# Limeth/euclider

Hardware: NVIDIA B200
Metric: Mrays/s (higher is better)
Workload: dtype f64

## Files before the change

### euclider_b200/csrc/cuda/api_device.cu

```cuda
#include <algorithm>
#include <cmath>
#include <cstdio>
#include <cstdlib>
#include <cstring>
#include <condition_variable>
#include <functional>
#include <mutex>
#include <string>
#include <thread>
#include <vector>

#include "error.h"
#include "euclider_b200.h"
#include "intersect.cuh"
#include "pipeline.cuh"
#include "scene_dev.cuh"

namespace {

using namespace eucl;

#define EUCL_CUDA(expr)                                                                                   \
    do {                                                                                                  \
        cudaError_t _e = (expr);                                                                          \
// ... 53 lines not shown
            }
        });
    }
    void run(std::function<void()> f) {
        std::lock_guard<std::mutex> lk(m);
        job = std::move(f);
        has_job = true;
        done = false;
        cv.notify_all();
    }
    void wait() {
        std::unique_lock<std::mutex> lk(m);
        cv.wait(lk, [this] { return done; });
    }
    void stop() {
        if (!th.joinable()) return;
        {
            std::lock_guard<std::mutex> lk(m);
            quit = true;
            cv.notify_all();
        }
        th.join();
    }
};

}

struct EuclScene {
    int device = 0;
    int dim = 3;
    int sm_count = 148;
    int blob_bytes = 0;
    size_t smem_bytes = 0;
    size_t smem_scene = 0;
    unsigned long long shade_light_mask = 1ull, shade_heavy_mask = 0ull;
    uint8_t* d_blob = nullptr;
    std::vector<cudaArray_t> arrays;
    std::vector<cudaTextureObject_t> tex_objects;
    cudaStream_t stream = nullptr;
    cudaStream_t own_stream = nullptr;
    cudaEvent_t ev[2] = {nullptr, nullptr};
    cudaStream_t side_stream = nullptr;
    cudaEvent_t ev_fork = nullptr, ev_join = nullptr;
    std::vector<cudaEvent_t> prof_events;
    DeviceBuffer nodes;
    DeviceBuffer small;
    DeviceBuffer frame;
    DeviceBuffer hit_ids;
    DeviceBuffer order;
    DeviceBuffer path_io;
    DeviceBuffer rorder;
    int n_cull = 0;
    int light_capable = 0;
    int ray_bins_mode = -1;
    bool ray_bins_now = true;
    float tune_ms[2] = {0.f, 0.f};
    int tune_count[2] = {0, 0};
    uint64_t tune_pixels = 0;
    int warm_frames = 0;
    int n_entities = 0;
    int real_bytes = 8;
    int arena_capacity = 0;
    double arena_factor = 0.0;
    cudaGraphExec_t graph_exec = nullptr;
    uint64_t graph_key = 0, seen_key = 0;
    uint32_t graph_launches = 0;
    int list_capacity = 0;
    double list_factor = 1.0;
    int32_t* h_small = nullptr;
    std::vector<EuclScene*> twins;
    std::vector<Worker*> workers;
    bool is_twin = false;
    cudaEvent_t ev_split[3] = {nullptr, nullptr, nullptr};
    cudaEvent_t ev_done = nullptr;
};

namespace {

constexpr int kSmallInts = 4 * (EUCL_MAX_LEVELS + 1) + 16 + (EUCL_MAX_LEVELS + 1) * (kMaxBins + kRayBins);
struct SmallLayout {
    static constexpr int count = 0;
    static constexpr int level_off = EUCL_MAX_LEVELS + 1;
    static constexpr int overflow = 2 * (EUCL_MAX_LEVELS + 1);
    static constexpr int cam_entity = overflow + 1;
    static constexpr int undefined64 = overflow + 2;
    static constexpr int mega64 = undefined64 + 2;
    static constexpr int bins = mega64 + 2 * (EUCL_MAX_LEVELS + 1);
    static constexpr int rbins = bins + (EUCL_MAX_LEVELS + 1) * kMaxBins;
    static constexpr int total = rbins + (EUCL_MAX_LEVELS + 1) * kRayBins;
};
static_assert(SmallLayout::undefined64 % 2 == 0, "u64 counters must be 8-byte aligned");
static_assert(SmallLayout::total <= kSmallInts, "small buffer layout");

size_t align16(size_t v) { return (v + 15) & ~size_t(15); }

int validate_scene(const EuclFlatScene& f, std::string* why) {
    auto bad = [&](const std::string& msg) {
        *why = msg;
        return (int)EUCL_ERR_INVALID_ARGUMENT;
    };
    const int counts[] = {f.n_prims, f.n_nodes, f.n_entities, f.n_materials, f.n_transforms, f.n_expr_ops,
                          f.n_surfaces, f.n_color_ops, f.n_mapped_textures, f.n_textures};
    for (int c : counts)
        if (c < 0) return bad("negative table size");
    if ((f.n_prims && !f.prims) || (f.n_nodes && !f.nodes) || (f.n_entities && !f.entities) || (f.n_materials && !f.materials) ||
        (f.n_transforms && !f.transforms) || (f.n_expr_ops && !f.expr_ops) || (f.n_surfaces && !f.surfaces) ||
// ... 561 lines not shown
        for (int k = 0; k < EUCL_MAX_DIM; ++k) planes[(size_t)i * kPlaneStride + k] = flat->prims[i].v0[k];
        planes[(size_t)i * kPlaneStride + 4] = flat->prims[i].s0;
        planes[(size_t)i * kPlaneStride + 5] = flat->prims[i].s1;
    }
    h.off_planes = w.put(planes.data(), planes.size());
    MacroBuilder mb{*flat, {}};
    std::vector<EuclEntity> dev_entities((size_t)flat->n_entities);
    std::vector<char> negated((size_t)std::max(flat->n_entities, 1), 0);
    for (int e = 0; e < flat->n_entities; ++e) {
        EuclEntity de = flat->entities[e];
        de.node_first = (int)mb.out.size();
        const int root = flat->entities[e].node_root;
        const EuclNode& rn = flat->nodes[root];
        if (rn.op == EUCL_CSG_COMPLEMENT && flat->nodes[mb.child_a(root)].op == EUCL_CSG_LEAF &&
            flat->prims[flat->nodes[mb.child_a(root)].prim].kind == EUCL_PRIM_VOID && env_int("EUCL_NEGATED_ROOMS", 1)) {
            negated[(size_t)e] = 1;
            mb.emit(mb.child_b(root));
        } else {
            mb.emit(root);
        }
        de.node_root = (int)mb.out.size() - 1;
        int peak = 0, depth = 0;
        if (!mb.fits(de.node_first, de.node_root, &peak, &depth))
            return bail(EUCL_ERR_SCENE_LIMIT, "entity " + std::to_string(e) + ": CSG program too large for the device evaluator (" +
                                                  std::to_string(peak) + " arena slots of " + std::to_string(CSG_ARENA) + ", nesting " +
                                                  std::to_string(depth) + ")");
        dev_entities[(size_t)e] = de;
    }
    std::vector<Bound> bounds(mb.out.size());
    for (int e = 0; e < flat->n_entities; ++e)
        mb.compute_bounds(dev_entities[(size_t)e].node_first, dev_entities[(size_t)e].node_root, s->real_bytes == 4 ? 1e-3 : 1e-6, &bounds);
    if (!env_int("EUCL_BOUND_CULL", 1))
        for (auto& b : bounds) b.r2 = -1.0;
    h.n_nodes = (int)mb.out.size();
    h.off_nodes = w.put(mb.out.data(), mb.out.size());
    h.off_bounds = w.put(bounds.data(), bounds.size());
    for (int e = 0; e < flat->n_entities && h.n_cull < 4; ++e) {
        const EuclEntity& de = dev_entities[(size_t)e];
        if (de.surface >= 0 && !negated[(size_t)e] && mb.out[(size_t)de.node_root].kind != M_PRIM && bounds[(size_t)de.node_root].r2 >= 0.0)
            h.cull_root[h.n_cull++] = de.node_root;
    }
    s->n_cull = h.n_cull;
    std::vector<int32_t> ent_flags((size_t)std::max(flat->n_entities, 1), 0);
    bool light_capable = true;
    for (int e = 0; e < flat->n_entities; ++e) {
        const EuclEntity& de = dev_entities[(size_t)e];
        if (negated[(size_t)e]) ent_flags[(size_t)e] = ENT_NEGATED;
        if (de.surface < 0) continue;
        const MNode& root = mb.out[(size_t)de.node_root];
        int fl = ENT_SURFACED | ent_flags[(size_t)e];
        if (root.kind == M_PRIM) fl |= ENT_PRIM;
        else if (root.kind == M_CHAIN && de.node_first == de.node_root && (root.b & 0x4000) && (root.b & 0x3fff) <= kPlaneChainMax) fl |= ENT_ROOT_PLANES;
        for (int k = 0; k < h.n_cull; ++k)
            if (h.cull_root[k] == de.node_root) fl |= ENT_CULL_ROOT;
        if (!(fl & (ENT_PRIM | ENT_ROOT_PLANES | ENT_CULL_ROOT))) light_capable = false;
        ent_flags[(size_t)e] = fl;
    }
    if (!env_int("EUCL_INTERSECT_SPLIT", 1)) light_capable = false;
    h.light_capable = light_capable ? 1 : 0;
    s->light_capable = h.light_capable;
    h.off_ent_flags = w.put(ent_flags.data(), ent_flags.size());
    h.off_entities = w.put(dev_entities.data(), dev_entities.size());
    h.off_materials = w.put(flat->materials, (size_t)flat->n_materials);
    h.off_transforms = w.put(flat->transforms, (size_t)flat->n_transforms);
    h.off_expr_ops = w.put(flat->expr_ops, (size_t)flat->n_expr_ops);
    std::vector<LinRow> lin_rows((size_t)std::max(flat->n_transforms, 1) * 2 * EUCL_MAX_DIM);
    for (int t = 0; t < flat->n_transforms; ++t)
        for (int k = 0; k < flat->dim; ++k) {
            const EuclTransform& tr = flat->transforms[t];
            lin_rows[(size_t)t * 2 * EUCL_MAX_DIM + k] = lower_lin_row(flat->expr_ops + tr.fwd_first[k], tr.fwd_len[k], flat->dim);
            lin_rows[(size_t)t * 2 * EUCL_MAX_DIM + EUCL_MAX_DIM + k] = lower_lin_row(flat->expr_ops + tr.inv_first[k], tr.inv_len[k], flat->dim);
        }
    h.off_lin_rows = w.put(lin_rows.data(), lin_rows.size());
    h.off_surfaces = w.put(flat->surfaces, (size_t)flat->n_surfaces);
    h.off_color_ops = w.put(flat->color_ops, (size_t)flat->n_color_ops);
    h.off_mapped = w.put(flat->mapped_textures, (size_t)flat->n_mapped_textures);
    h.off_textures = w.put(flat->textures, (size_t)flat->n_textures);
    h.off_tex_objects = w.put(s->tex_objects.data(), s->tex_objects.size());
    h.off_perlin = w.put(flat->perlin_perm, 256);
    int max_nodes = 1;
    for (int e = 0; e < flat->n_entities; ++e)
        max_nodes = std::max(max_nodes, flat->entities[e].node_root - flat->entities[e].node_first + 1);
    h.max_entity_nodes = max_nodes;
    h.blob_bytes = (int)w.bytes.size();
    std::memcpy(w.bytes.data(), &h, sizeof h);
    s->blob_bytes = h.blob_bytes;
    s->smem_scene = scene_smem_bytes(h.blob_bytes);
    s->smem_bytes = s->smem_scene + sizeof(double) * kPlaneChainMax * kBlock;
    s->shade_light_mask = 1ull;
    s->shade_heavy_mask = 0ull;
    if (kBinsPerEntity * flat->n_entities + 1 <= kMaxBins)
        for (int e = 0; e < flat->n_entities; ++e) {
            const int sf = flat->entities[e].surface;
            if (sf < 0) continue;
            const bool simple = flat->surfaces[sf].ratio_op == EUCL_RATIO_UNIFORM && flat->surfaces[sf].thr_op == EUCL_THR_IDENTITY;
            const unsigned long long bits = ((1ull << kBinsPerEntity) - 1ull) << (1 + kBinsPerEntity * e);
            (simple ? s->shade_light_mask : s->shade_heavy_mask) |= bits;
        }
    if (env_int("EUCL_SHADE_SPLIT", 1) == 0) {
        s->shade_heavy_mask |= s->shade_light_mask;
        s->shade_light_mask = 0ull;
    }
    int smem_optin = 0;
    cudaDeviceGetAttribute(&smem_optin, cudaDevAttrMaxSharedMemoryPerBlockOptin, device);
    if (s->smem_bytes > (size_t)smem_optin)
        return bail(EUCL_ERR_SCENE_LIMIT, "scene tables (" + std::to_string(s->smem_bytes) +
                                              " B) exceed the shared memory of one CTA (" + std::to_string(smem_optin) + " B)");
    EUCL_CUDA_S(cudaMalloc((void**)&s->d_blob, w.bytes.size()));
    EUCL_CUDA_S(cudaMemcpy(s->d_blob, w.bytes.data(), w.bytes.size(), cudaMemcpyHostToDevice));
    EUCL_CUDA_S(EUCL_PREC(configure_kernels)(s->smem_bytes, s->smem_scene));
    EUCL_CUDA_S(cudaMallocHost((void**)&s->h_small, sizeof(int32_t) * kSmallInts));
#undef EUCL_CUDA_S
    *out = s;
// ... 88 lines not shown
    return ws;
}

void choose_grouping(EuclScene* s) {
    const int forced = env_int("EUCL_BIN_RAYS", -1);
    if (forced >= 0) s->ray_bins_mode = forced ? 1 : 0;
    if (s->ray_bins_mode >= 0) s->ray_bins_now = s->ray_bins_mode == 1;
    else s->ray_bins_now = s->tune_count[1] <= s->tune_count[0];
}

void tune_grouping(EuclScene* s, const EuclStats& st, int pipeline) {
    if (s->ray_bins_mode >= 0 || st.retries != 0 || st.pixels == 0 || pipeline != EUCL_PIPELINE_WAVEFRONT) return;
    if (s->n_cull == 0) {
        s->ray_bins_mode = 0;
    } else if (s->warm_frames >= 1) {
        if (s->tune_pixels != st.pixels) {
            s->tune_pixels = st.pixels;
            s->tune_ms[0] = s->tune_ms[1] = 0.f;
            s->tune_count[0] = s->tune_count[1] = 0;
        }
        const int m = s->ray_bins_now ? 1 : 0;
        s->tune_ms[m] = s->tune_count[m] == 0 ? st.ms_total : std::min(s->tune_ms[m], st.ms_total);
        s->tune_count[m] += 1;
        if (s->tune_count[0] >= 2 && s->tune_count[1] >= 2) s->ray_bins_mode = s->tune_ms[1] < s->tune_ms[0] ? 1 : 0;
    }
}

int render_impl(EuclScene* s, const EuclCamera* cam, const EuclRenderOpts* o, uint8_t* d_rgb, int32_t* d_hit,
                EuclStats* stats, int sub_stride = 1, int sub_offset = 0) {
    const int dim = s->dim;
    FrameParams fp;
    frame_params(*cam, *o, s->real_bytes, &fp);
    const int width = (int)o->width;
    const uint32_t my_rows = eucl_band_rows_for_rank(o);
    EuclStats st{};
    st.levels = cam->max_depth + 1;
    if (!s->is_twin) choose_grouping(s);
    EUCL_CUDA(cudaEventRecord(s->ev[0], s->stream));
    if (my_rows > 0) {
        const long long chunk_pixels_target = std::max(1, env_int("EUCL_CHUNK_PIXELS", 1 << 25));
        int rows_per_chunk = (int)std::max<long long>(1, chunk_pixels_target / width);
        rows_per_chunk = std::min<int>(rows_per_chunk, (int)my_rows);
        if ((long long)width > (1ll << 30)) return fail(EUCL_ERR_INVALID_ARGUMENT, "frame rows too wide");
        EUCL_CUDA(s->small.ensure(sizeof(int32_t) * kSmallInts));
        if (s->arena_factor <= 0.0) s->arena_factor = std::max(1.0, (double)env_int("EUCL_ARENA_FACTOR_X10", 45) / 10.0);
        Launch l{s->stream, s->d_blob, s->smem_bytes, s->smem_scene,
                 s->sm_count * std::max(1, env_int("EUCL_BLOCKS_PER_SM", kResidentThreads / kBlock)),
                 s->sm_count * std::max(1, env_int("EUCL_LIGHT_BLOCKS_PER_SM", kLightResidentBlocks)),
                 s->sm_count * std::max(1, env_int("EUCL_SHADE_BLOCKS_PER_SM", kShadeResidentBlocks)),
                 s->sm_count * std::max(1, env_int("EUCL_MEM_BLOCKS_PER_SM", 8)),
                 s->shade_light_mask, s->shade_heavy_mask,
                 s->sm_count * std::max(1, env_int("EUCL_LIGHT_K2_BLOCKS_PER_SM", kLightK2ResidentBlocks)), s->light_capable, s->n_cull,
                 (o->profile || env_int("EUCL_DEBUG_SYNC", 0) || !env_int("EUCL_CONCURRENT", 1)) ? nullptr : s->side_stream, s->ev_fork,
                 s->ev_join, s->sm_count * std::max(1, env_int("EUCL_BACKGROUND_BLOCKS_PER_SM", EUCL_BACKGROUND_MIN_BLOCKS))};
        const bool want_rorder = o->pipeline == EUCL_PIPELINE_WAVEFRONT && s->n_cull > 0 && env_int("EUCL_BIN_RAYS", 1);
        const bool want_order = o->pipeline == EUCL_PIPELINE_WAVEFRONT && kBinsPerEntity * s->n_entities + 1 <= kMaxBins && env_int("EUCL_BIN_SHADE", 1);
        const size_t n_lists = (want_rorder ? (size_t)kRayBins : 0) + (want_order ? (size_t)(kBinsPerEntity * s->n_entities + 1) : 0);
        auto workspace_bytes = [&](size_t cap, size_t list_cap) { return arena_bytes(dim, s->real_bytes, cap) + sizeof(int32_t) * n_lists * list_cap; };

        for (int row0 = 0; row0 < (int)my_rows;) {
            ChunkParams cp{};
            cp.local_row0 = row0;
            cp.band_rows = o->band_rows ? (int)o->band_rows : (int)o->height;
            cp.band_rank = (int)o->band_rank;
            cp.band_world = o->band_world ? (int)o->band_world : 1;
            cp.compact_rows = o->compact_rows;
            cp.sub_stride = sub_stride;
            cp.sub_offset = sub_offset;
            for (;;) {
                cp.n_rows = std::min<int>(rows_per_chunk, (int)my_rows - row0);
                cp.n_pixels = cp.n_rows * width;
                long long want = (long long)std::ceil((double)rows_per_chunk * (double)width * s->arena_factor) + 1024;
                if (o->pipeline == EUCL_PIPELINE_MEGAKERNEL) want = 16;
                long long want_list = (long long)std::ceil((double)rows_per_chunk * (double)width * s->list_factor) + 1024;
                if (o->pipeline == EUCL_PIPELINE_MEGAKERNEL) want_list = 16;
                bool too_big = want > 0x7fff0000ll || want_list > 0x7fff0000ll;
                if (!too_big && ((int)want > s->arena_capacity || (int)want_list > s->list_capacity)) {
                    EUCL_CUDA(cudaStreamSynchronize(s->stream));
                    want = std::max<long long>(want, s->arena_capacity);
                    want_list = std::max<long long>(want_list, s->list_capacity);
                    size_t free_b = 0, total_b = 0;
                    EUCL_CUDA(cudaMemGetInfo(&free_b, &total_b));
                    const size_t held = s->nodes.bytes + s->order.bytes + s->rorder.bytes;
                    size_t budget = (size_t)((double)(free_b + held) * 0.85);
                    const int cap_mb = env_int("EUCL_ARENA_MAX_MB", 0);
                    if (cap_mb > 0) budget = std::min(budget, (size_t)cap_mb << 20);
                    too_big = workspace_bytes((size_t)want, (size_t)want_list) > budget;
                    if (!too_big) {
                        cudaError_t e = s->nodes.ensure(arena_bytes(dim, s->real_bytes, (size_t)want));
                        if (e == cudaSuccess && want_rorder) e = s->rorder.ensure(sizeof(int32_t) * (size_t)kRayBins * (size_t)want_list);
                        if (e == cudaSuccess && want_order) e = s->order.ensure(sizeof(int32_t) * (size_t)(kBinsPerEntity * s->n_entities + 1) * (size_t)want_list);
                        if (e == cudaSuccess) {
                            s->arena_capacity = (int)want;
                            s->list_capacity = (int)want_list;
                        } else {
                            cudaGetLastError();
                            s->nodes.release();
                            s->rorder.release();
                            s->order.release();
                            s->arena_capacity = 0;
                            s->list_capacity = 0;
                            if (e != cudaErrorMemoryAllocation) return fail(EUCL_ERR_CUDA, std::string("workspace allocation: ") + cudaGetErrorString(e));
                            too_big = true;
                        }
                    }
                }
                if (too_big) {
// ... 27 lines not shown
                    return fail(EUCL_ERR_SCENE_LIMIT, "megakernel pipeline supports max_depth <= 24");
                auto enqueue = [&]() -> uint32_t {
                    uint32_t launches = 0;
                    cudaMemsetAsync(s->small.ptr, 0, sizeof(int32_t) * kSmallInts, s->stream);
                    if (poison) {
                        cudaMemsetAsync(s->nodes.ptr, 0x7F, s->nodes.bytes, s->stream);
                        if (s->order.ptr) cudaMemsetAsync(s->order.ptr, 0x7F, s->order.bytes, s->stream);
                        if (s->rorder.ptr) cudaMemsetAsync(s->rorder.ptr, 0x7F, s->rorder.bytes, s->stream);
                    }
                    mark(-1);
                    if (o->pipeline == EUCL_PIPELINE_MEGAKERNEL) {
                        EUCL_PREC(launch_camera_entity)(dim, l, fp, ws);
                        dbg("k_camera_entity", 0);
                        EUCL_PREC(launch_megakernel)(dim, l, fp, cp, ws, d_rgb, d_hit);
                        mark(1);
                        launches += 2;
                    } else {
                        EUCL_PREC(launch_raygen)(dim, l, fp, cp, ws, d_hit);
                        dbg("k_raygen", 0);
                        mark(0);
                        for (int level = 0; level < (int)cam->max_depth; ++level) {
                            launches += EUCL_PREC(launch_intersect)(dim, l, ws, level);
                            dbg("k_intersect", level);
                            mark(1);
                            launches += EUCL_PREC(launch_shade)(dim, l, fp, cp, ws, level, d_hit);
                            dbg("k_shade", level);
                            mark(2);
                        }
                        launches += EUCL_PREC(launch_shade)(dim, l, fp, cp, ws, (int)cam->max_depth, d_hit);
                        dbg("k_shade", (int)cam->max_depth);
                        mark(2);
                        launches += EUCL_PREC(launch_resolve_and_final)(dim, l, fp, cp, ws, d_rgb);
                        dbg("k_resolve / k_final", 0);
                        mark(3);
                        launches += 1;
                    }
                    cudaMemcpyAsync(s->h_small, s->small.ptr, sizeof(int32_t) * kSmallInts, cudaMemcpyDeviceToHost, s->stream);
                    return launches;
                };
                uint64_t key = 1469598103934665603ull;
                auto mix = [&](const void* data, size_t bytes) {
                    const unsigned char* b = (const unsigned char*)data;
                    for (size_t k = 0; k < bytes; ++k) key = (key ^ b[k]) * 1099511628211ull;
                };
                mix(&fp, sizeof fp);
                mix(&cp, sizeof cp);
                mix(&ws, sizeof ws);
                {
                    const void* ptrs[] = {l.stream, l.blob, l.side};
                    const unsigned long long nums[] = {l.smem_bytes, l.smem_scene, (unsigned long long)l.grid_max, (unsigned long long)l.grid_light,
                                                       (unsigned long long)l.grid_shade, (unsigned long long)l.grid_mem, l.shade_light_mask,
                                                       l.shade_heavy_mask, (unsigned long long)l.grid_light_k2,
                                                       (unsigned long long)l.light_capable, (unsigned long long)l.n_cull,
                                                       (unsigned long long)l.grid_background};
                    mix(ptrs, sizeof ptrs);
                    mix(nums, sizeof nums);
                }
                mix(&d_rgb, sizeof d_rgb);
                mix(&d_hit, sizeof d_hit);
                const int pipeline_id = o->pipeline;
                mix(&pipeline_id, sizeof pipeline_id);
                const uint32_t depth_id = cam->max_depth;
                mix(&depth_id, sizeof depth_id);
                const bool graph_ok = env_int("EUCL_GRAPH", 1) && !o->profile && !debug_sync && !poison &&
                                      (s->ray_bins_mode >= 0 || o->pipeline != EUCL_PIPELINE_WAVEFRONT);
                if (graph_ok && s->graph_exec && s->graph_key == key) {
                    EUCL_CUDA(cudaGraphLaunch(s->graph_exec, s->stream));
                    st.launches += s->graph_launches;
                    st.graph_replays += 1;
                } else if (graph_ok && s->seen_key == key) {
                    if (s->graph_exec) cudaGraphExecDestroy(s->graph_exec);
                    s->graph_exec = nullptr;
                    cudaGraph_t graph = nullptr;
                    static std::mutex capture_mutex;
                    std::unique_lock<std::mutex> capture_lock(capture_mutex);
                    EUCL_CUDA(cudaStreamBeginCapture(s->stream, cudaStreamCaptureModeThreadLocal));
                    const uint32_t launches = enqueue();
                    cudaError_t ce = cudaStreamEndCapture(s->stream, &graph);
                    if (ce == cudaSuccess) ce = cudaGraphInstantiate(&s->graph_exec, graph, 0);
                    capture_lock.unlock();
                    if (graph) cudaGraphDestroy(graph);
                    if (ce != cudaSuccess) {
                        cudaGetLastError();
                        s->graph_exec = nullptr;
                        s->seen_key = 0;
                        st.launches += enqueue();
                    } else {
                        s->graph_key = key;
                        s->graph_launches = launches;
                        EUCL_CUDA(cudaGraphLaunch(s->graph_exec, s->stream));
                        st.launches += launches;
                        st.graph_replays += 1;
                    }
                } else {
                    s->seen_key = key;
                    st.launches += enqueue();
                }
                if (!fault.empty()) return fail(EUCL_ERR_CUDA, "EUCL_DEBUG_SYNC: " + fault);
                EUCL_CUDA(cudaStreamSynchronize(s->stream));
                EUCL_CUDA(cudaGetLastError());
                for (size_t k = 1; k < prof_family.size(); ++k) {
                    float ms = 0.f;
                    cudaEventElapsedTime(&ms, s->prof_events[k - 1], s->prof_events[k]);
                    float* slot = prof_family[k] == 0 ? &st.ms_raygen : prof_family[k] == 1 ? &st.ms_intersect
                                  : prof_family[k] == 2 ? &st.ms_shade : &st.ms_resolve;
                    *slot += ms;
                }
// ... 33 lines not shown
            const bool traced = s->h_small[SmallLayout::cam_entity] >= 0;
            for (uint32_t lv = 0; traced && lv <= cam->max_depth; ++lv) {
                uint64_t c = o->pipeline == EUCL_PIPELINE_MEGAKERNEL
                                 ? ((const unsigned long long*)(s->h_small + SmallLayout::mega64))[lv]
                                 : (uint64_t)s->h_small[SmallLayout::count + lv];
                st.level_counts[lv] += c;
                st.nodes += c;
                if (lv < cam->max_depth) st.segments += c;
            }
        }
    }
    EUCL_CUDA(cudaEventRecord(s->ev[1], s->stream));
    EUCL_CUDA(cudaEventSynchronize(s->ev[1]));
    EUCL_CUDA(cudaEventElapsedTime(&st.ms_total, s->ev[0], s->ev[1]));
    if (st.retries > 0 && st.pixels > 0 && st.nodes > 0 && o->pipeline == EUCL_PIPELINE_WAVEFRONT && st.pixels == (uint64_t)my_rows * width) {
        uint64_t max_level = 0;
        for (uint32_t lv = 0; lv <= cam->max_depth; ++lv) max_level = std::max<uint64_t>(max_level, st.level_counts[lv]);
        const double tight = (double)st.nodes / (double)st.pixels * 1.03 + 0.02;
        const double tight_list = std::max(1.0, (double)max_level / (double)st.pixels * 1.03);
        if ((double)s->arena_capacity > ((double)st.pixels * tight + 1024) * 1.08) {
            s->arena_factor = tight;
            s->list_factor = tight_list;
            s->nodes.release();
            s->order.release();
            s->rorder.release();
            s->arena_capacity = 0;
            s->list_capacity = 0;
            if (s->graph_exec) cudaGraphExecDestroy(s->graph_exec);
            s->graph_exec = nullptr;
            s->graph_key = s->seen_key = 0;
        }
    }
    if (sub_stride <= 1) tune_grouping(s, st, o->pipeline);
    s->warm_frames++;
    st.ray_grouping = s->ray_bins_now && s->rorder.ptr != nullptr && o->pipeline == EUCL_PIPELINE_WAVEFRONT ? 1u : 0u;
    if (stats) *stats = st;
    return EUCL_OK;
}

int add_twin(EuclScene* s) {
    EuclScene* t = new EuclScene();
    t->is_twin = true;
    t->device = s->device;
    t->dim = s->dim;
    t->sm_count = s->sm_count;
    t->blob_bytes = s->blob_bytes;
    t->smem_bytes = s->smem_bytes;
    t->smem_scene = s->smem_scene;
    t->shade_light_mask = s->shade_light_mask;
    t->shade_heavy_mask = s->shade_heavy_mask;
    t->d_blob = s->d_blob;
    t->n_cull = s->n_cull;
    t->light_capable = s->light_capable;
    t->n_entities = s->n_entities;
    t->real_bytes = s->real_bytes;
    cudaError_t e = cudaStreamCreateWithFlags(&t->own_stream, cudaStreamNonBlocking);
    t->stream = t->own_stream;
    if (e == cudaSuccess) e = cudaEventCreate(&t->ev[0]);
    if (e == cudaSuccess) e = cudaEventCreate(&t->ev[1]);
    if (e == cudaSuccess) e = cudaStreamCreateWithFlags(&t->side_stream, cudaStreamNonBlocking);
    if (e == cudaSuccess) e = cudaEventCreateWithFlags(&t->ev_fork, cudaEventDisableTiming);
    if (e == cudaSuccess) e = cudaEventCreateWithFlags(&t->ev_join, cudaEventDisableTiming);
    if (e == cudaSuccess) e = cudaEventCreateWithFlags(&t->ev_done, cudaEventDisableTiming);
    if (e == cudaSuccess) e = cudaMallocHost((void**)&t->h_small, sizeof(int32_t) * kSmallInts);
    for (int k = 0; k < 3 && e == cudaSuccess; ++k)
        if (!s->ev_split[k]) e = cudaEventCreateWithFlags(&s->ev_split[k], k == 1 ? cudaEventDisableTiming : cudaEventDefault);
    if (e != cudaSuccess) {
        cudaGetLastError();
        eucl_scene_destroy(t);
        return fail(e == cudaErrorMemoryAllocation ? EUCL_ERR_OUT_OF_MEMORY : EUCL_ERR_CUDA, std::string("split pipeline: ") + cudaGetErrorString(e));
    }
    s->twins.push_back(t);
    s->workers.push_back(new Worker());
    s->workers.back()->start();
    return EUCL_OK;
}

constexpr int kMaxSplit = 8;

int render_split(EuclScene* s, const EuclCamera* cam, const EuclRenderOpts* o, uint8_t* d_rgb, int32_t* d_hit, EuclStats* stats) {
    const uint32_t my_rows = eucl_band_rows_for_rank(o);
    uint32_t world = o->band_world > 1 ? o->band_world : 1, rank = world > 1 ? o->band_rank : 0, band = o->band_rows;
    if (band == 0) {
        world = 1;
        rank = 0;
        band = (uint32_t)std::max(1, env_int("EUCL_SPLIT_BAND_ROWS", 16));
    }
    int k = std::min(kMaxSplit, env_int("EUCL_SPLIT", EUCL_SPLIT_DEFAULT));
    k = (int)std::min<uint32_t>((uint32_t)std::max(k, 1), my_rows / band);
    if (o->pipeline != EUCL_PIPELINE_WAVEFRONT || (long long)my_rows * o->width < (long long)env_int("EUCL_SPLIT_MIN_PIXELS", 1 << 16)) k = 1;
    if (k <= 1) return render_impl(s, cam, o, d_rgb, d_hit, stats);
    while ((int)s->twins.size() < k - 1) {
        int rc = add_twin(s);
        if (rc != EUCL_OK) return rc;
    }
    choose_grouping(s);
    EuclRenderOpts opts[kMaxSplit];
    EuclStats part[kMaxSplit];
    int rc[kMaxSplit];
    std::string err[kMaxSplit];
    for (int p = 0; p < k; ++p) {
        opts[p] = *o;
        opts[p].band_rows = band;
        opts[p].band_world = (uint32_t)k * world;
        opts[p].band_rank = rank + (uint32_t)p * world;
        part[p] = EuclStats{};
// ... 238 lines not shown
```

### euclider_b200/csrc/cuda/intersect.cuh

```cuda
#pragma once
#include "scene_dev.cuh"
#include "vecmath.cuh"

namespace EUCL_NS {
using namespace eucl;

#ifndef EUCL_CSG_ARENA
#define EUCL_CSG_ARENA 256
#endif
constexpr int CSG_ARENA = EUCL_CSG_ARENA;
constexpr int CSG_LIST_STACK = 16;
constexpr int CHAIN_ROOT_CAP = 32;

struct CHit {
    real t;
    int prim;
    int flags;
};

__device__ __forceinline__ int quadratic_hits(real a, real b, real c, real& t_first, real& t_second) {
    real disc = b * b - R(4.0) * a * c;
    if (disc < R(0.0)) return 0;
    real d_sqrt = sqrt(disc);
    real t1 = (-b - d_sqrt) / (R(2.0) * a);
// ... 477 lines not shown
                } else if (in) {
                    hb.flags ^= 2;
                }
                arena[out0 + outn++] = hb;
            }
        }
        for (int k = 0; k < outn; ++k) arena[a0 + k] = arena[out0 + k];
        top = a0 + outn;
        lstart[sp] = a0;
        llen[sp] = outn;
        ++sp;
    }
    if (llen[0] > 0) {
        out = arena[lstart[0]];
        return true;
    }
    return false;
}

struct ClosestHit {
    int entity;
    int prim;
    int flags;
    real t;
};

template <int D>
__device__ __forceinline__ ClosestHit closest_hit(const SceneView& sv, const Vec<D>& o, const Vec<D>& d, real* ts,
                                                  int ts_stride) {
    ClosestHit best{-1, 0, 0, R(0.0)};
    const real dd = dot(d, d);
    for (int e = 0; e < sv.n_entities; ++e) {
        const EuclEntity ent = sv.entities()[e];
        if (ent.surface < 0) continue;
        CHit h;
        bool found;
        const MNode root = reinterpret_cast<const MNode*>(sv.nodes())[ent.node_root];
        if (root.kind != M_PRIM && ray_misses<D>(sv.bounds()[ent.node_root], o, d, dd)) continue;
        if (root.kind == M_PRIM) {
            real t0 = R(0.0), t1 = R(0.0);
            found = prim_roots<D>(sv, root.a, o, d, t0, t1) > 0;
            h = CHit{t0, root.a, 0};
        } else {
            found = csg_first<D>(sv, ent.node_first, ent.node_root, o, d, ts, ts_stride, h);
        }
        if (sv.ent_flags()[e] & ENT_NEGATED) h.flags ^= 2;
        if (found && (best.entity < 0 || best.t > h.t)) best = ClosestHit{e, h.prim, h.flags, h.t};
    }
    return best;
}

template <int D>
__device__ __forceinline__ ClosestHit closest_hit_light(const SceneView& sv, const Vec<D>& o, const Vec<D>& d, real* ts,
                                                        int ts_stride) {
    ClosestHit best{-1, 0, 0, R(0.0)};
    for (int e = 0; e < sv.n_entities; ++e) {
        const int flags = sv.ent_flags()[e];
        if (!(flags & ENT_SURFACED) || (flags & ENT_CULL_ROOT)) continue;
        const MNode root = reinterpret_cast<const MNode*>(sv.nodes())[sv.entities()[e].node_root];
        real t0 = R(0.0), t1 = R(0.0);
        int prim = root.a;
        bool found;
        if (flags & ENT_PRIM) {
            found = prim_roots<D>(sv, root.a, o, d, t0, t1) > 0;
        } else {
            unsigned long long L = 0ull;
            found = plane_chain<D>(sv, root.b >> 16, root.a, root.b & 0x3fff, o, d, true, ts, ts_stride, L) > 0;
            const int idx = (int)(L & 15ull);
            t0 = ts[idx * ts_stride];
            prim = root.a + idx;
        }
        if (found && (best.entity < 0 || best.t > t0)) best = ClosestHit{e, prim, (flags & ENT_NEGATED) ? 2 : 0, t0};
    }
    return best;
}

template <int D>
__device__ __forceinline__ void hit_geometry(const SceneView& sv, int prim, int flags, const Vec<D>& o, const Vec<D>& d,
                                             real t, Vec<D>& p, Vec<D>& nrm) {
    const int n = sv.n_prims;
    const int kind = sv.prim_kind()[prim];
    if (kind == EUCL_PRIM_SPHERE) {
        p = o + d * t;
        nrm = normalize(p - load_vec<D>(sv.prim_v0() + prim, n));
    } else if (kind == EUCL_PRIM_CYLINDER) {
        Vec<D> center = load_vec<D>(sv.prim_v0() + prim, n);
        Vec<D> axis = load_vec<D>(sv.prim_v1() + prim, n);
        real t_first = t;
        if (flags & 1) {
            real r0 = R(0.0), r1 = R(0.0);
            prim_roots<D>(sv, prim, o, d, r0, r1);
            t_first = r0;
        }
        Vec<D> p1 = o + d * t_first;
        Vec<D> on_axis = axis * dot(axis, p1 - center) + center;
        p = o + d * t;
        nrm = normalize(p - on_axis);
    } else {
        p = d * t + o;
        nrm = load_vec<D>(sv.prim_v0() + prim, n);
        if (kind == EUCL_PRIM_HALFSPACE) nrm = nrm * -R(sv.prim_s1()[prim]);
    }
    if (flags & 2) nrm = -nrm;
}

}
```

### euclider_b200/csrc/cuda/kernels.cu

```cuda
#include "pipeline.cuh"
#include "shade.cuh"
#include <cstdio>
#include <cstdlib>

namespace EUCL_NS {
using namespace eucl;

namespace {

#ifndef EUCL_INTERSECT_MIN_BLOCKS
#define EUCL_INTERSECT_MIN_BLOCKS (kResidentThreads / kBlock)
#endif


constexpr int kWordReals = 16 / (int)sizeof(real);
struct __align__(16) Word {
    real v[kWordReals];
};
template <int N>
__device__ __forceinline__ void store_words(void* base, size_t record, const real (&v)[N]) {
    Word* rec = reinterpret_cast<Word*>(base) + record * (N / kWordReals);
#pragma unroll
    for (int k = 0; k < N / kWordReals; ++k) {
        Word w;
// ... 316 lines not shown
    __shared__ int s_skip, s_total;
    __shared__ int s_rprefix[kRayBins + 1];
    const int off = ws.level_off[level], cnt = ws.count[level];
    const bool grouped = ws.ray_bins != 0;
    __shared__ int s_rcount[kRayBins];
    if (threadIdx.x < kRayBins)
        s_rcount[threadIdx.x] = (grouped && ((key_mask >> threadIdx.x) & 1u)) ? ws.rbin_count[level * kRayBins + threadIdx.x] : 0;
    if (threadIdx.x == 32)
        s_skip = *ws.overflow != 0 || *ws.cam_entity < 0;
    __syncthreads();
    if (threadIdx.x == 0) {
        int acc = cnt;
        if (grouped) {
            acc = 0;
            for (int b = 0; b < kRayBins; ++b) {
                s_rprefix[b] = acc;
                acc += s_rcount[b];
            }
            s_rprefix[kRayBins] = acc;
        }
        s_total = acc;
        if (blockIdx.x == 0) ws.level_off[level + 1] = off + cnt;
    }
    __syncthreads();
    const int total = s_total;
    if (s_skip || (int)(blockIdx.x * blockDim.x) >= total) return;
    const SceneView& sv = stage_scene(blob);
    real* ts = plane_scratch(blob);
    const unsigned lane = threadIdx.x & 31u;
    const int stride = gridDim.x * blockDim.x;
    const int first = warp_first_position();
    int bin = 0;
    auto node_at = [&](int i) -> int {
        if (i >= total) return -1;
        if (!grouped) return off + i;
        while (i >= s_rprefix[bin + 1]) ++bin;
        return ws.rorder[(size_t)bin * ws.list_cap + (i - s_rprefix[bin])];
    };
    int node_next = node_at(first + (int)lane);
    for (int base = first; base < total; base += stride) {
        int node = node_next;
        node_next = node_at(base + stride + (int)lane);
        bool valid = node >= 0;
        if (grouped && valid && (node < off || node >= off + cnt)) {
            *ws.overflow = 2;
            valid = false;
        }
        int ent = -1;
        bool exiting_flag = false;
        real cos_hint = R(0.0);
        if (valid) {
            Vec<D> o, d;
            load_ray<D>(ws, node, o, d);
            const ClosestHit h = LIGHT ? closest_hit_light<D>(sv, o, d, ts, (int)blockDim.x) : closest_hit<D>(sv, o, d, ts, (int)blockDim.x);
            HitHead rec{R(0.0), R(0.0), R(0.0), -1, 0};
            Vec<D> n;
#pragma unroll
            for (int k = 0; k < D; ++k) n[k] = R(0.0);
            if (h.entity >= 0) {
                Vec<D> p;
                hit_geometry<D>(sv, h.prim, h.flags, o, d, h.t, p, n);
                const real cos_raw = angle_cos(d, n);
                const real angle_raw = angle_from_cos(cos_raw);
                const bool exiting = angle_raw < kFracPi2;
                rec = HitHead{h.t, cos_raw, angle_raw, h.entity, exiting ? 1 : 0};
                exiting_flag = exiting;
                cos_hint = cos_raw;
            }
            ent = h.entity;
            store_hit<D>(ws, node, rec, n);
        }
        if (ws.n_bins > 1) {
            const unsigned active = __ballot_sync(0xffffffffu, valid);
            if (valid) {
                int cls = exiting_flag ? 1 : 0;
                if (exiting_flag && ent >= 0) {
                    const EuclSurface& sf = sv.surfaces()[sv.entities()[ent].surface];
                    if (sf.ratio_op == EUCL_RATIO_FRESNEL) {
                        if (R(sf.ratio_a) * R(sf.ratio_a) * (R(1.0) - cos_hint * cos_hint) > R(sf.ratio_b) * R(sf.ratio_b)) cls = 2;
                    }
                }
                const int key = ent < 0 ? 0 : 1 + kBinsPerEntity * ent + cls;
                const unsigned peers = __match_any_sync(active, key);
                const int leader = __ffs(peers) - 1;
                int slot = 0;
                if ((int)lane == leader) slot = atomicAdd(&ws.bin_count[level * kMaxBins + key], __popc(peers));
                slot = __shfl_sync(peers, slot, leader);
                ws.order[(size_t)key * ws.list_cap + slot + __popc(peers & ((1u << lane) - 1u))] = node;
            }
        }
    }
}

template <int D, bool RAY_BINS, bool GLASS>
__global__ void __launch_bounds__(GLASS ? kShadeBlock : kLightBlock, GLASS ? EUCL_SHADE_MIN_BLOCKS : EUCL_SHADE_LIGHT_MIN_BLOCKS)
    k_shade(const uint8_t* __restrict__ blob, FrameParams fp, ChunkParams cp, Workspace ws, int level, unsigned long long bin_mask,
            int32_t* __restrict__ hit_ids_out) {
    const int off = ws.level_off[level], cnt = ws.count[level];
    const bool last_level = level >= fp.max_depth;
    __shared__ int s_prefix[kMaxBins + 1];
    __shared__ int s_skip, s_total;
    const bool binned = ws.n_bins > 1 && !last_level;
    __shared__ int s_bcount[kMaxBins];
    if (threadIdx.x < kMaxBins)
        s_bcount[threadIdx.x] = (binned && (int)threadIdx.x < ws.n_bins && ((bin_mask >> threadIdx.x) & 1ull))
                                    ? ws.bin_count[level * kMaxBins + threadIdx.x] : 0;
    if (threadIdx.x == 64) s_skip = level > 0 && *ws.overflow != 0;
// ... 386 lines not shown
        } else {
            a0 = __fma_rn(a0, m, c); a1 = __fma_rn(a1, m, c); a2 = __fma_rn(a2, m, c); a3 = __fma_rn(a3, m, c);
            a4 = __fma_rn(a4, m, c); a5 = __fma_rn(a5, m, c); a6 = __fma_rn(a6, m, c); a7 = __fma_rn(a7, m, c);
        }
    }
    out[blockIdx.x * blockDim.x + threadIdx.x] = ((a0 + a1) + (a2 + a3)) + ((a4 + a5) + (a6 + a7));
}

#endif
inline int grid_for(int n, int block, int grid_max) {
    long long g = ((long long)n + block - 1) / block;
    if (g < 1) g = 1;
    if (g > grid_max) g = grid_max;
    return (int)g;
}

}

#define EUCL_DISPATCH_DIM(dim, CALL3, CALL4) \
    do {                                     \
        if ((dim) == 3) { CALL3; }           \
        else { CALL4; }                      \
    } while (0)

void launch_camera_entity(int dim, const Launch& l, const FrameParams& fp, const Workspace& ws) {
    EUCL_DISPATCH_DIM(dim, (k_camera_entity<3><<<1, 32, l.smem_scene, l.stream>>>(l.blob, fp, ws)),
                      (k_camera_entity<4><<<1, 32, l.smem_scene, l.stream>>>(l.blob, fp, ws)));
}
void launch_raygen(int dim, const Launch& l, const FrameParams& fp, const ChunkParams& cp, const Workspace& ws,
                   int32_t* hit_ids_out) {
    const int grid = grid_for(cp.n_pixels, kBlock, l.grid_mem);
    EUCL_DISPATCH_DIM(dim, (k_raygen<3><<<grid, kBlock, l.smem_scene, l.stream>>>(l.blob, fp, cp, ws, hit_ids_out)),
                      (k_raygen<4><<<grid, kBlock, l.smem_scene, l.stream>>>(l.blob, fp, cp, ws, hit_ids_out)));
}
static void fork_side(const Launch& l) {
    cudaEventRecord(l.ev_fork, l.stream);
    cudaStreamWaitEvent(l.side, l.ev_fork, 0);
}
static void join_side(const Launch& l) {
    cudaEventRecord(l.ev_join, l.side);
    cudaStreamWaitEvent(l.stream, l.ev_join, 0);
}

int launch_intersect(int dim, const Launch& l, const Workspace& ws, int level) {
    const bool light_all = l.light_capable && l.n_cull == 0;
    const bool split = l.light_capable && ws.ray_bins != 0;
    const size_t smem_light = l.smem_scene + sizeof(real) * kPlaneChainMax * kLightK2Block;
    const bool light = light_all || split, heavy = !light_all;
    const bool fork = light && heavy && l.side != nullptr;
    cudaStream_t light_stream = fork ? l.side : l.stream;
    if (fork) fork_side(l);
    int launches = 0;
    if (light) {
        EUCL_DISPATCH_DIM(dim, (k_intersect<3, true><<<l.grid_light_k2, kLightK2Block, smem_light, light_stream>>>(l.blob, ws, level, 1u)),
                          (k_intersect<4, true><<<l.grid_light_k2, kLightK2Block, smem_light, light_stream>>>(l.blob, ws, level, 1u)));
        ++launches;
    }
    if (heavy) {
        const unsigned mask = split ? 0xfffeu : 0xffffu;
        EUCL_DISPATCH_DIM(dim, (k_intersect<3, false><<<l.grid_max, kBlock, l.smem_bytes, l.stream>>>(l.blob, ws, level, mask)),
                          (k_intersect<4, false><<<l.grid_max, kBlock, l.smem_bytes, l.stream>>>(l.blob, ws, level, mask)));
        ++launches;
    }
    if (fork) join_side(l);
    return launches;
}
template <int D, bool RAY_BINS, bool GLASS>
static void launch_shade_one(const Launch& l, cudaStream_t stream, const FrameParams& fp, const ChunkParams& cp, const Workspace& ws,
                             int level, unsigned long long mask, int32_t* hit_ids_out) {
    if (GLASS) k_shade<D, RAY_BINS, true><<<l.grid_shade, kShadeBlock, l.smem_scene, stream>>>(l.blob, fp, cp, ws, level, mask, hit_ids_out);
    else k_shade<D, RAY_BINS, false><<<l.grid_light, kLightBlock, l.smem_scene, stream>>>(l.blob, fp, cp, ws, level, mask, hit_ids_out);
}
template <int D, bool GLASS>
static void launch_shade_dim(const Launch& l, cudaStream_t stream, const FrameParams& fp, const ChunkParams& cp, const Workspace& ws,
                             int level, unsigned long long mask, int32_t* hit_ids_out) {
    if (ws.ray_bins && level + 1 < fp.max_depth) launch_shade_one<D, true, GLASS>(l, stream, fp, cp, ws, level, mask, hit_ids_out);
    else launch_shade_one<D, false, GLASS>(l, stream, fp, cp, ws, level, mask, hit_ids_out);
}
int launch_shade(int dim, const Launch& l, const FrameParams& fp, const ChunkParams& cp, const Workspace& ws, int level,
                 int32_t* hit_ids_out) {
    const bool last_level = level >= fp.max_depth;
    unsigned long long light = l.shade_light_mask, heavy = l.shade_heavy_mask;
    if (last_level) {
        const int grid = l.grid_background;
        EUCL_DISPATCH_DIM(dim, (k_background<3><<<grid, 256, l.smem_scene, l.stream>>>(l.blob, fp, cp, ws, level, hit_ids_out)),
                          (k_background<4><<<grid, 256, l.smem_scene, l.stream>>>(l.blob, fp, cp, ws, level, hit_ids_out)));
        return 1;
    } else if (ws.n_bins <= 1) {
        light = 0ull;
        heavy = ~0ull;
    }
    int launches = 0;
    const bool fork = light && heavy && l.side != nullptr;
    cudaStream_t light_stream = fork ? l.side : l.stream;
    if (fork) fork_side(l);
    if (light) {
        EUCL_DISPATCH_DIM(dim, (launch_shade_dim<3, false>(l, light_stream, fp, cp, ws, level, light, hit_ids_out)),
                          (launch_shade_dim<4, false>(l, light_stream, fp, cp, ws, level, light, hit_ids_out)));
        ++launches;
    }
    if (heavy) {
        EUCL_DISPATCH_DIM(dim, (launch_shade_dim<3, true>(l, l.stream, fp, cp, ws, level, heavy, hit_ids_out)),
                          (launch_shade_dim<4, true>(l, l.stream, fp, cp, ws, level, heavy, hit_ids_out)));
        ++launches;
    }
    if (fork) join_side(l);
    return launches;
}
int launch_resolve_and_final(int dim, const Launch& l, const FrameParams& fp, const ChunkParams& cp, const Workspace& ws,
                             uint8_t* out_rgb8) {
    (void)dim;
    int launches = 0;
// ... 106 lines not shown
```

### euclider_b200/csrc/cuda/pipeline.cuh

```cuda
#pragma once
#include <cuda_runtime.h>
#include <stdint.h>

#include "euclider_b200.h"

namespace eucl {

struct FrameParams {
    double location[EUCL_MAX_DIM];
    double center[EUCL_MAX_DIM];
    double up[EUCL_MAX_DIM];
    double right[EUCL_MAX_DIM];
    double time_millis;
    int32_t width, height;
    int32_t max_depth;
    int32_t _pad;
};

struct ChunkParams {
    int32_t local_row0;
    int32_t n_rows;
    int32_t band_rows, band_rank, band_world;
    int32_t compact_rows;
    int32_t n_pixels;
// ... 20 lines not shown
    double ratio;
    int32_t tchild;
    int32_t rchild;
    uint32_t q;
    uint32_t flags;
};
enum : uint32_t {
    NODE_LEAF = 1u,
    NODE_HAS_SC = 2u,
    NODE_FINAL_RGB = 4u,
    NODE_UNDEFINED = 8u
};

struct Workspace {
    int32_t capacity;
    int32_t list_cap;
    void* ray;
    int32_t* ray_cur;
    void* hit;
    NodeMeta* meta;
    void* res;
    int32_t* count;
    int32_t* level_off;
    int32_t* overflow;
    int32_t* cam_entity;
    int32_t n_bins;
    int32_t _pad2;
    int32_t* bin_count;
    int32_t* order;
    int32_t ray_bins;
    int32_t _pad3;
    int32_t* rbin_count;
    int32_t* rorder;
    unsigned long long* undefined_count;
    unsigned long long* mega_level_counts;
};

struct Launch {
    cudaStream_t stream;
    const uint8_t* blob;
    size_t smem_bytes;
    size_t smem_scene;
    int grid_max;
    int grid_light;
    int grid_shade;
    int grid_mem;
    unsigned long long shade_light_mask, shade_heavy_mask;
    int grid_light_k2;
    int light_capable;
    int n_cull;
    cudaStream_t side;
    cudaEvent_t ev_fork, ev_join;
    int grid_background;
};

#ifndef EUCL_BLOCK
#define EUCL_BLOCK 512
#endif
constexpr int kBlock = EUCL_BLOCK;
constexpr int kResidentThreads = 512;
#ifndef EUCL_LIGHT_BLOCK
#define EUCL_LIGHT_BLOCK 256
#endif
#ifndef EUCL_BACKGROUND_MIN_BLOCKS
#define EUCL_BACKGROUND_MIN_BLOCKS 3
#endif
#ifndef EUCL_SHADE_LIGHT_MIN_BLOCKS
#define EUCL_SHADE_LIGHT_MIN_BLOCKS 2
#endif
#ifndef EUCL_SHADE_BLOCK
#define EUCL_SHADE_BLOCK EUCL_BLOCK
#endif
#ifndef EUCL_SHADE_MIN_BLOCKS
#define EUCL_SHADE_MIN_BLOCKS (512 / EUCL_SHADE_BLOCK > 0 ? 512 / EUCL_SHADE_BLOCK : 1)
#endif
constexpr int kShadeBlock = EUCL_SHADE_BLOCK;
constexpr int kShadeResidentBlocks = EUCL_SHADE_MIN_BLOCKS;
constexpr int kLightBlock = EUCL_LIGHT_BLOCK;
constexpr int kLightResidentBlocks = EUCL_SHADE_LIGHT_MIN_BLOCKS;
#ifndef EUCL_LIGHT_K2_BLOCK
#define EUCL_LIGHT_K2_BLOCK 128
#endif
#ifndef EUCL_INTERSECT_LIGHT_MIN_BLOCKS
#define EUCL_INTERSECT_LIGHT_MIN_BLOCKS 5
#endif
constexpr int kLightK2Block = EUCL_LIGHT_K2_BLOCK;
constexpr int kLightK2ResidentBlocks = EUCL_INTERSECT_LIGHT_MIN_BLOCKS;
constexpr int kRayBins = 16;
constexpr int kBinsPerEntity = 3;
constexpr int kMaxBins = 64;

}

#define EUCL_DECLARE_LAUNCHERS(NS)                                                                                             \
    namespace NS {                                                                                                             \
    void launch_camera_entity(int dim, const eucl::Launch& l, const eucl::FrameParams& fp, const eucl::Workspace& ws);        \
    void launch_raygen(int dim, const eucl::Launch& l, const eucl::FrameParams& fp, const eucl::ChunkParams& cp,              \
                       const eucl::Workspace& ws, int32_t* hit_ids_out);                                                       \
    int launch_intersect(int dim, const eucl::Launch& l, const eucl::Workspace& ws, int level);                                \
    int launch_shade(int dim, const eucl::Launch& l, const eucl::FrameParams& fp, const eucl::ChunkParams& cp,                \
                     const eucl::Workspace& ws, int level, int32_t* hit_ids_out);                                              \
    int launch_resolve_and_final(int dim, const eucl::Launch& l, const eucl::FrameParams& fp, const eucl::ChunkParams& cp,    \
                                 const eucl::Workspace& ws, uint8_t* out_rgb8);                                                \
    void launch_megakernel(int dim, const eucl::Launch& l, const eucl::FrameParams& fp, const eucl::ChunkParams& cp,          \
                           const eucl::Workspace& ws, uint8_t* out_rgb8, int32_t* hit_ids_out);                                \
    void launch_trace_path(int dim, const eucl::Launch& l, const double* d_in, double distance, double* d_out, int* d_found); \
// ... 8 lines not shown
```

### euclider_b200/csrc/cuda/scene_dev.cuh

```cuda
#pragma once
#include <cuda_runtime.h>
#include <stdint.h>

#include "euclider_b200.h"

namespace eucl {

struct SceneHeader {
    int32_t dim;
    int32_t n_prims, n_nodes, n_entities, n_materials, n_transforms, n_expr_ops;
    int32_t n_surfaces, n_color_ops, n_mapped_textures, n_textures;
    int32_t background;
    int32_t max_entity_nodes;
    int32_t blob_bytes;
    int32_t off_prim_kind, off_prim_v0, off_prim_v1, off_prim_s0, off_prim_s1;
    int32_t off_nodes, off_entities, off_materials, off_transforms, off_expr_ops;
    int32_t off_surfaces, off_color_ops, off_mapped, off_textures, off_tex_objects, off_perlin;
    int32_t off_planes, off_bounds;
    int32_t n_cull;
    int32_t cull_root[4];
    int32_t off_ent_flags;
    int32_t light_capable;
    int32_t off_lin_rows;
};

constexpr int kLinTermsMax = 4;
struct LinTerm {
    int32_t var;
    int32_t kind;
    double c;
};
struct LinRow {
    int32_t n_terms;
    int32_t _pad;
    LinTerm t[kLinTermsMax];
};
static_assert(sizeof(LinRow) % 8 == 0, "LinRow alignment");

enum EntFlags : int32_t {
    ENT_SURFACED = 1,
    ENT_PRIM = 2,
    ENT_ROOT_PLANES = 4,
    ENT_CULL_ROOT = 8,
    ENT_NEGATED = 16
};
static_assert(sizeof(SceneHeader) % 16 == 0, "header must keep 16-byte alignment");

struct Bound {
    double c[EUCL_MAX_DIM];
    double r2;
    double _pad;
};

#if defined(__CUDACC__)
extern __shared__ __align__(16) unsigned char g_smem[];
#endif

struct SceneView {
    int dim, n_prims, n_nodes, n_entities, n_surfaces, background;
    int n_cull, cull_root[4];
    uint32_t o_prim_kind, o_prim_v0, o_prim_v1, o_prim_s0, o_prim_s1, o_planes, o_nodes, o_entities, o_materials,
        o_transforms, o_expr_ops, o_surfaces, o_color_ops, o_mapped, o_textures, o_tex_objects, o_perlin, o_bounds, o_ent_flags, o_lin_rows;
#if defined(__CUDACC__)
#define EUCL_TABLE(type, name) \
    __device__ __forceinline__ const type* name() const { return reinterpret_cast<const type*>(g_smem + o_##name); }
    EUCL_TABLE(int32_t, prim_kind)
    EUCL_TABLE(double, prim_v0)
    EUCL_TABLE(double, prim_v1)
    EUCL_TABLE(double, prim_s0)
    EUCL_TABLE(double, prim_s1)
    EUCL_TABLE(double, planes)
    EUCL_TABLE(EuclNode, nodes)
    EUCL_TABLE(EuclEntity, entities)
    EUCL_TABLE(EuclMaterial, materials)
    EUCL_TABLE(EuclTransform, transforms)
    EUCL_TABLE(EuclExprOp, expr_ops)
    EUCL_TABLE(EuclSurface, surfaces)
    EUCL_TABLE(EuclColorOp, color_ops)
    EUCL_TABLE(EuclMappedTexture, mapped)
    EUCL_TABLE(EuclTexture, textures)
    EUCL_TABLE(cudaTextureObject_t, tex_objects)
    EUCL_TABLE(uint8_t, perlin)
    EUCL_TABLE(Bound, bounds)
    EUCL_TABLE(int32_t, ent_flags)
    EUCL_TABLE(LinRow, lin_rows)
#undef EUCL_TABLE
#endif
};
constexpr int kExprStackMax = 16;
constexpr int kColorStackMax = 8;
constexpr int kPlaneStride = 6;

#if defined(__CUDACC__)
__device__ __forceinline__ const SceneView& stage_scene(const uint8_t* __restrict__ blob) {
    SceneView* view = reinterpret_cast<SceneView*>(g_smem);
    const uint32_t base = (uint32_t)((sizeof(SceneView) + 15) & ~size_t(15));
    unsigned char* dst = g_smem + base;
// ... 48 lines not shown
```

Baseline: 3310.

## Route ray bins whose cull-root hits are plane chains to the light intersect kernel

Stores each entity's cull-root index in its flags. For ray bins whose only enabled cull roots are plane-chain roots, the bin is now handled by the light intersect kernel, which tests those roots inline instead of skipping all cull-root entities. This moves more rays off the heavy general intersect kernel. In exchange, each light-kernel thread does a short linear search of the bin prefix array to find its bin key, and correctness depends on the plane-chain path matching the heavy path for those entities.

New measurement: 3296 (median of 6 runs). No clear change (-0.4%).

```diff
diff --git a/euclider_b200/csrc/cuda/api_device.cu b/euclider_b200/csrc/cuda/api_device.cu
--- a/euclider_b200/csrc/cuda/api_device.cu
+++ b/euclider_b200/csrc/cuda/api_device.cu
@@ -129,6 +129,7 @@
     DeviceBuffer rorder;
     int n_cull = 0;
     int light_capable = 0;
+    unsigned light_key_mask = 1u;
     int ray_bins_mode = -1;
     bool ray_bins_now = true;
     float tune_ms[2] = {0.f, 0.f};
@@ -796,13 +797,21 @@
         if (root.kind == M_PRIM) fl |= ENT_PRIM;
         else if (root.kind == M_CHAIN && de.node_first == de.node_root && (root.b & 0x4000) && (root.b & 0x3fff) <= kPlaneChainMax) fl |= ENT_ROOT_PLANES;
         for (int k = 0; k < h.n_cull; ++k)
-            if (h.cull_root[k] == de.node_root) fl |= ENT_CULL_ROOT;
+            if (h.cull_root[k] == de.node_root) fl |= ENT_CULL_ROOT | (k << ENT_CULL_SHIFT);
         if (!(fl & (ENT_PRIM | ENT_ROOT_PLANES | ENT_CULL_ROOT))) light_capable = false;
         ent_flags[(size_t)e] = fl;
     }
     if (!env_int("EUCL_INTERSECT_SPLIT", 1)) light_capable = false;
     h.light_capable = light_capable ? 1 : 0;
     s->light_capable = h.light_capable;
+    unsigned chain_bits = 0u;
+    for (int e = 0; e < flat->n_entities; ++e)
+        if ((ent_flags[(size_t)e] & (ENT_CULL_ROOT | ENT_ROOT_PLANES)) == (ENT_CULL_ROOT | ENT_ROOT_PLANES))
+            chain_bits |= 1u << ((ent_flags[(size_t)e] >> ENT_CULL_SHIFT) & 3);
+    if (!env_int("EUCL_LIGHT_CHAIN_KEYS", 1)) chain_bits = 0u;
+    s->light_key_mask = 0u;
+    for (unsigned key = 0; key < (unsigned)kRayBins; ++key)
+        if ((key & ~chain_bits) == 0u) s->light_key_mask |= 1u << key;
     h.off_ent_flags = w.put(ent_flags.data(), ent_flags.size());
     h.off_entities = w.put(dev_entities.data(), dev_entities.size());
     h.off_materials = w.put(flat->materials, (size_t)flat->n_materials);
@@ -997,7 +1006,8 @@
                  s->shade_light_mask, s->shade_heavy_mask,
                  s->sm_count * std::max(1, env_int("EUCL_LIGHT_K2_BLOCKS_PER_SM", kLightK2ResidentBlocks)), s->light_capable, s->n_cull,
                  (o->profile || env_int("EUCL_DEBUG_SYNC", 0) || !env_int("EUCL_CONCURRENT", 1)) ? nullptr : s->side_stream, s->ev_fork,
-                 s->ev_join, s->sm_count * std::max(1, env_int("EUCL_BACKGROUND_BLOCKS_PER_SM", EUCL_BACKGROUND_MIN_BLOCKS))};
+                 s->ev_join, s->sm_count * std::max(1, env_int("EUCL_BACKGROUND_BLOCKS_PER_SM", EUCL_BACKGROUND_MIN_BLOCKS)),
+                 s->light_key_mask};
         const bool want_rorder = o->pipeline == EUCL_PIPELINE_WAVEFRONT && s->n_cull > 0 && env_int("EUCL_BIN_RAYS", 1);
         const bool want_order = o->pipeline == EUCL_PIPELINE_WAVEFRONT && kBinsPerEntity * s->n_entities + 1 <= kMaxBins && env_int("EUCL_BIN_SHADE", 1);
         const size_t n_lists = (want_rorder ? (size_t)kRayBins : 0) + (want_order ? (size_t)(kBinsPerEntity * s->n_entities + 1) : 0);
@@ -1131,7 +1141,7 @@
                                                        (unsigned long long)l.grid_shade, (unsigned long long)l.grid_mem, l.shade_light_mask,
                                                        l.shade_heavy_mask, (unsigned long long)l.grid_light_k2,
                                                        (unsigned long long)l.light_capable, (unsigned long long)l.n_cull,
-                                                       (unsigned long long)l.grid_background};
+                                                       (unsigned long long)l.grid_background, (unsigned long long)l.light_key_mask};
                     mix(ptrs, sizeof ptrs);
                     mix(nums, sizeof nums);
                 }
@@ -1271,6 +1281,7 @@
     t->d_blob = s->d_blob;
     t->n_cull = s->n_cull;
     t->light_capable = s->light_capable;
+    t->light_key_mask = s->light_key_mask;
     t->n_entities = s->n_entities;
     t->real_bytes = s->real_bytes;
     cudaError_t e = cudaStreamCreateWithFlags(&t->own_stream, cudaStreamNonBlocking);
diff --git a/euclider_b200/csrc/cuda/intersect.cuh b/euclider_b200/csrc/cuda/intersect.cuh
--- a/euclider_b200/csrc/cuda/intersect.cuh
+++ b/euclider_b200/csrc/cuda/intersect.cuh
@@ -553,11 +553,17 @@
 
 template <int D>
 __device__ __forceinline__ ClosestHit closest_hit_light(const SceneView& sv, const Vec<D>& o, const Vec<D>& d, real* ts,
-                                                        int ts_stride) {
+                                                        int ts_stride, const int* rprefix, int pos) {
     ClosestHit best{-1, 0, 0, R(0.0)};
     for (int e = 0; e < sv.n_entities; ++e) {
         const int flags = sv.ent_flags()[e];
-        if (!(flags & ENT_SURFACED) || (flags & ENT_CULL_ROOT)) continue;
+        if (!(flags & ENT_SURFACED)) continue;
+        if (flags & ENT_CULL_ROOT) {
+            int key = 0;
+            if (rprefix)
+                while (pos >= rprefix[key + 1]) ++key;
+            if (!((key >> ((flags >> ENT_CULL_SHIFT) & 3)) & 1)) continue;
+        }
         const MNode root = reinterpret_cast<const MNode*>(sv.nodes())[sv.entities()[e].node_root];
         real t0 = R(0.0), t1 = R(0.0);
         int prim = root.a;
diff --git a/euclider_b200/csrc/cuda/kernels.cu b/euclider_b200/csrc/cuda/kernels.cu
--- a/euclider_b200/csrc/cuda/kernels.cu
+++ b/euclider_b200/csrc/cuda/kernels.cu
@@ -392,7 +392,7 @@
         if (valid) {
             Vec<D> o, d;
             load_ray<D>(ws, node, o, d);
-            const ClosestHit h = LIGHT ? closest_hit_light<D>(sv, o, d, ts, (int)blockDim.x) : closest_hit<D>(sv, o, d, ts, (int)blockDim.x);
+            const ClosestHit h = LIGHT ? closest_hit_light<D>(sv, o, d, ts, (int)blockDim.x, grouped ? s_rprefix : nullptr, base + (int)lane) : closest_hit<D>(sv, o, d, ts, (int)blockDim.x);
             HitHead rec{R(0.0), R(0.0), R(0.0), -1, 0};
             Vec<D> n;
 #pragma unroll
@@ -885,12 +885,12 @@
     if (fork) fork_side(l);
     int launches = 0;
     if (light) {
-        EUCL_DISPATCH_DIM(dim, (k_intersect<3, true><<<l.grid_light_k2, kLightK2Block, smem_light, light_stream>>>(l.blob, ws, level, 1u)),
-                          (k_intersect<4, true><<<l.grid_light_k2, kLightK2Block, smem_light, light_stream>>>(l.blob, ws, level, 1u)));
+        EUCL_DISPATCH_DIM(dim, (k_intersect<3, true><<<l.grid_light_k2, kLightK2Block, smem_light, light_stream>>>(l.blob, ws, level, l.light_key_mask)),
+                          (k_intersect<4, true><<<l.grid_light_k2, kLightK2Block, smem_light, light_stream>>>(l.blob, ws, level, l.light_key_mask)));
         ++launches;
     }
     if (heavy) {
-        const unsigned mask = split ? 0xfffeu : 0xffffu;
+        const unsigned mask = split ? 0xffffu & ~l.light_key_mask : 0xffffu;
         EUCL_DISPATCH_DIM(dim, (k_intersect<3, false><<<l.grid_max, kBlock, l.smem_bytes, l.stream>>>(l.blob, ws, level, mask)),
                           (k_intersect<4, false><<<l.grid_max, kBlock, l.smem_bytes, l.stream>>>(l.blob, ws, level, mask)));
         ++launches;
diff --git a/euclider_b200/csrc/cuda/pipeline.cuh b/euclider_b200/csrc/cuda/pipeline.cuh
--- a/euclider_b200/csrc/cuda/pipeline.cuh
+++ b/euclider_b200/csrc/cuda/pipeline.cuh
@@ -96,6 +96,7 @@
     cudaStream_t side;
     cudaEvent_t ev_fork, ev_join;
     int grid_background;
+    unsigned light_key_mask;
 };
 
 #ifndef EUCL_BLOCK
diff --git a/euclider_b200/csrc/cuda/scene_dev.cuh b/euclider_b200/csrc/cuda/scene_dev.cuh
--- a/euclider_b200/csrc/cuda/scene_dev.cuh
+++ b/euclider_b200/csrc/cuda/scene_dev.cuh
@@ -42,7 +42,8 @@
     ENT_PRIM = 2,
     ENT_ROOT_PLANES = 4,
     ENT_CULL_ROOT = 8,
-    ENT_NEGATED = 16
+    ENT_NEGATED = 16,
+    ENT_CULL_SHIFT = 8
 };
 static_assert(sizeof(SceneHeader) % 16 == 0, "header must keep 16-byte alignment");
 
```
